# timfpark/heatmap

Hardware: AMD Instinct MI355X
Metric: points binned/sec (whole node, zooms 0-18) + % HBM roofline at 1/2/4/8 GPU (higher is better)
Workload: dtype f64

## Files before the change

heatmap_amd/csrc/hm_api.cpp:

```cpp
#include <hip/hip_runtime.h>
#include <stdio.h>
#include <stdlib.h>
#include <string.h>

#include <math.h>

#include <algorithm>
#include <chrono>
#include <vector>

#include "hm_genkey.h"
#include "hm_ctx.h"

namespace {

struct Level {
    int zc;
    int dbits;
    uint32_t nparents;
    uint64_t nchildren;
    uint32_t count = 0;
    uint32_t items = 0;
    bool out16 = false;
};
// ... 526 lines not shown
    *L = l;
}

namespace {

struct LevelOut {
    void* keys = nullptr;
    int slot_k = 0;
    HmRuns runs = {nullptr, nullptr};
    const uint32_t* parent_item_begin = nullptr;
    const uint64_t* parent_coord = nullptr;
    uint32_t nparents = 1;
    uint64_t level_keys = 0;
    uint32_t* seg = nullptr;
};

struct Level1Work {
    HmPart1Args a;
    uint32_t *rbase, *rcap;
    uint8_t* smask;
    HmL1Args ba;
    int F;
    uint32_t* hist;
    int64_t *redo_rows, *redo_cols;
    uint64_t stride;
    uint64_t total_cap;
    void* kout;
};

struct LevelWork {
    int restbits;
    bool contig;
    bool hot3;
    int sb;
    uint64_t l1_total;
    void* kout;
    uint2* runs_sh;
    uint32_t* nruns;
    uint32_t* rs_big;
    HmRsArgs ra;
    uint64_t* prefix;
};

struct CountCall {
    hm_ctx* ctx;
    const double* lat;
    const double* lon;
    const int64_t* rows;
    const int64_t* cols;
    const uint8_t* keep;
    int64_t n;
    int zmin, Z;
    uint64_t* keys_out;
    uint64_t* counts_out;
    int64_t capacity;
    int64_t* n_out;
    int64_t* xcells_out;
    int64_t xcapacity;
    int64_t* nx_out;

    hipStream_t s = nullptr;
    int zb = 0;
    int zs[HM_MAX_LEVELS];
    int L = 0;
    uint32_t ta = HM_TA;
    bool timing = false;
    uint32_t tiles_in = 0;
    bool from_tiles = false;
    uint64_t redo_cap = 0;
    bool spread = false;

    LevelOut hand;

    bool hot_on = false;
    bool hot_mid = false;
    int hz = 0;
    uint32_t nhot = 0;
    uint64_t l2_elems = 0;
    HmHotRunArgs hr = {};

    Level lv[HM_MAX_LEVELS];
    HmBuckets B[HM_MAX_LEVELS] = {};
    unsigned long long* totals[HM_MAX_LEVELS + 1];
    uint32_t nslots = 0;
    int32_t* slots = nullptr;
    uint32_t* slot_bucket = nullptr;
    HmExotic xl = {};
    uint64_t nx = 0;
    HmOut o;

    int l1_reruns = 0;
    int npart = 0;
// ... 57 lines not shown
    s = ctx->stream;
    zb = Z > HM_AG_LG ? Z - HM_AG_LG : 0;
    hz = zb;
    {
        int z = zb < HM_Z1 ? zb : HM_Z1;
        zs[L++] = z;
        while (z < zb) {
            z = std::min(z + HM_LEVEL_ZOOMS, zb);
            if (L >= HM_MAX_LEVELS) return HM_E_ARG;
            zs[L++] = z;
        }
    }
    if (2 * (Z - zs[0]) > 32) return HM_E_ARG;
    timing = n >= (1ll << 24) && ctx->stage_timing;
    while (ta > ctx->ta_min && (uint64_t)n < (uint64_t)ta * ctx->ta_items) ta >>= 1;
    for (int i = 0; i < 9; i++) ctx->stage_us[i] = 0;
    ctx->stage_us[8] = (double)ta;
    ctx->last_levels = L;

    tiles_in = (uint32_t)((n + HM_T1 - 1) / HM_T1);
    from_tiles = rows != nullptr;
    redo_cap = from_tiles ? 0 : std::max<uint64_t>(1u << 20, (uint64_t)n / 256);
    if (redo_cap > (uint64_t)n) redo_cap = (uint64_t)n;
    xl.cap = std::min<uint64_t>((uint64_t)n, std::max<uint64_t>(1u << 20, (uint64_t)n / 256));
    ENSURE(B_X_ROW, xl.cap * 8 + 8, xl.row);
    ENSURE(B_X_COL, xl.cap * 8 + 8, xl.col);
    ENSURE(B_X_IDX, xl.cap * 8 + 8, xl.idx);
    xl.count = ctx->state + ST_XCOUNT;
    return HM_OK;
}

int CountCall::begin_level(int l)
{
    Level& V = lv[l];
    V.zc = zs[l];
    V.dbits = 2 * (zs[l] - (l ? zs[l - 1] : 0));
    V.nparents = hand.nparents;
    V.nchildren = (uint64_t)hand.nparents << V.dbits;
    V.out16 = (l == L - 1);
    if (V.nchildren > (uint64_t)HM_SCAN_LIMIT) return HM_FALLBACK;
    return HM_OK;
}

int CountCall::bucket_arrays(int l, uint64_t cap, HmCompactOut& out)
{
    ENSURE(B_BK0 + l * 8 + 0, cap * 4, out.nkeys);
// ... 54 lines not shown
    const Level& V = lv[0];
    HmFill f1;
    memset(&f1, 0, sizeof(f1));
    hm_fill_add(f1, ctx->state + 1, 0, (ST_COUNT - 1) * sizeof(unsigned long long));
    hm_fill_add(f1, ctx->state + ST_ERR, 0xFF, sizeof(unsigned long long));
    static_assert(ST_ERR == 0, "error word first");
    w.F = 1 << V.dbits;
    uint32_t* fill;
    ENSURE(B_L1_FILL, FS * 4, fill);
    ENSURE(B_L1_RBASE, FS * 4, w.rbase);
    ENSURE(B_L1_RCAP, FS * 4, w.rcap);
    ENSURE(B_L1_HIST, HM_D1 * 4, w.hist);
    ENSURE(B_L1_SMASK, HM_D1, w.smask);
    uint32_t* const hist = w.hist;
    uint4* l1slot = nullptr;
    if (!from_tiles) ENSURE(B_L1_SLOT, (size_t)FS * sizeof(uint4), l1slot);
    hot_mid = ctx->hot && ctx->hot_mid && L == 3 && zs[1] <= 11 && zs[0] == HM_Z1 && n > 0 && V.dbits == 2 * HM_Z1;
    hot_on = hot_mid || (ctx->hot && L == 2 && zb <= 11 && zs[0] == HM_Z1 && n > 0 && V.dbits == 2 * HM_Z1);
    hz = hot_mid ? zs[1] : zb;
    uint32_t* redo_idx = nullptr;
    w.redo_rows = w.redo_cols = nullptr;
    if (!from_tiles) {
        ENSURE(B_REDO_IDX, redo_cap * sizeof(uint32_t), redo_idx);
        ENSURE(B_REDO_ROWS, redo_cap * sizeof(int64_t), w.redo_rows);
        ENSURE(B_REDO_COLS, redo_cap * sizeof(int64_t), w.redo_cols);
    }
    HmPart1Args& a = w.a;
    memset(&a, 0, sizeof(a));
    a.lat = lat;
    a.lon = lon;
    a.rows_in = rows;
    a.cols_in = cols;
    a.keep = keep;
    a.n = n;
    a.Z = Z;
    a.dbits = V.dbits;
    a.restbits = 2 * (Z - zs[0]);
    a.fill = fill;
    a.rbase = w.rbase;
    a.rcap = w.rcap;
    a.smask = w.smask;
    a.l1slot = l1slot;
    a.overflow = ctx->state + ST_OVERFLOW;
    a.err_word = ctx->state + ST_ERR;
    a.x = xl;
    a.slow_count = ctx->state + ST_SLOW;
    a.redo_idx = redo_idx;
    a.redo_count = ctx->state + ST_REDO;
// ... 12 lines not shown
        ENSURE(B_HOT, (HM_MAX_HOT + HM_HOT_SLOTS + 2 * HM_HOT_CAND + 1) * 4, hot_tiles);
        ENSURE(B_HOT_PARENT, HM_MAX_F1, hot_parent);
        hot_hash = hot_tiles + HM_MAX_HOT;
        hm_fill_add(f1, hot_counts, 0, 4ull << (2 * hz));
        hm_fill_add(f1, hot_hash + HM_HOT_SLOTS + 2 * HM_HOT_CAND, 0, 4);
        hm_fill_add(f1, hot_parent, 0, HM_MAX_F1);
        a.hot_z = hz;
        a.hot_bytes = hot_mid ? 4 : 2;
        a.hot_hash = hot_hash;
        a.hot_n = hot_n;
    } else {
        a.hot_z = -1;
    }
    hm_launch_fill(s, f1);
    if (n > 0) hm_launch_sample_digits(s, a, stride, hist, hot_counts);
    HIPCHK(hipGetLastError());
    if (hot_on) {
        hr.tiles = hot_tiles;
        hr.n = hot_n;
        hr.zb = hz;
        hr.z1 = zs[0];
        hr.fill = fill;
        hr.rbase = w.rbase;
        HmHotArgs ha;
        ha.counts = hot_counts;
        ha.zb = hz;
        ha.z1 = zs[0];
        const uint64_t m = ((uint64_t)n + stride - 1) / stride;
        ha.thresh = (uint32_t)std::max<double>(
            {1.0, ceil((double)m / ctx->hot_inv_share), ceil(ctx->hot_min_keys / (double)stride)});
        ha.tiles = hot_tiles;
        ha.hist = hist;
        ha.hotparent = hot_parent;
        ha.n = hot_n;
        ha.hash = hot_hash;
        ha.cand = hot_hash + HM_HOT_SLOTS;
        hm_launch_hot_select(s, ha);
        HIPCHK(hipGetLastError());
    }
    return HM_OK;
}

int CountCall::level1_size(Level1Work& w)
{
    const HmPart1Args& a = w.a;
    const int F = w.F;
    const uint64_t stride = w.stride;
    int st;
    const double nn = (double)n + (double)(F + (hot_on ? HM_MAX_HOT : 0)) * (double)stride;
    const double M = F + std::min((double)F, nn / ((double)HM_L1_SHARD_TILES * HM_T1)) * (HM_L1_SHARDS - 1) +
                     (hot_on ? (double)HM_MAX_HOT * HM_L1_SHARDS : 0.0);
    double bound = nn * 17.0 / 16.0 + 8.0 * sqrt(M * nn * (double)stride) + M * 2.0 * HM_T1 +
                   (double)(F + (hot_on ? HM_MAX_HOT : 0)) * HM_L1_ZERO_SAMPLES * (double)stride + 1024.0;
    hm_launch_l1_sizes(s, w.hist, F, hot_on ? (uint32_t*)(ctx->state + ST_NHOT) : nullptr, stride, w.rcap, w.rbase,
                       w.smask, ctx->state + ST_L1TOTAL);
    if (a.l1slot) hm_launch_l1_slots(s, a);
    HIPCHK(hipGetLastError());
    if (bound >= (double)0xFFF00000ull) {
        if ((st = read_state(ctx))) return st;
        bound = (double)ctx->host_state[ST_L1TOTAL] + 1024.0;
        if (bound >= (double)0xFFF00000ull) return HM_FALLBACK;
    }
    w.total_cap = (uint64_t)bound;
    return HM_OK;
}

int CountCall::level1_bucket_args(Level1Work& w)
{
    const Level& V = lv[0];
    HmL1Args& ba = w.ba;
    int st;
    memset(&ba, 0, sizeof(ba));
    const uint64_t cap = (uint64_t)w.F + 1;
    if ((st = bucket_arrays(0, cap, ba.out))) return st;
    ENSURE(B_FLAT_A, (uint64_t)FS * sizeof(uint2) + 8, ba.runs);
    ENSURE(B_EXCL_A, (uint64_t)FS * sizeof(uint64_t) + 8, ba.excl);
    ENSURE(B_CHILD0, 2 * 4, ba.child_begin);
    ba.F = w.F;
    ba.dbits = V.dbits;
// ... 44 lines not shown
        }
    if (w.total_cap >= 0xFFF00000ull) return HM_FALLBACK;
    HIPCHK(hipMemcpyAsync(w.rcap, hc, FS * 4, hipMemcpyHostToDevice, s));
    HIPCHK(hipMemcpyAsync(w.rbase, hb, FS * 4, hipMemcpyHostToDevice, s));
    if (a.l1slot) hm_launch_l1_slots(s, a);
    return HM_OK;
}

int CountCall::level1_redo(Level1Work& w)
{
    HmRedoArgs ra;
    ra.lat = lat;
    ra.lon = lon;
    ra.keep = keep;
    ra.Z = Z;
    ra.redo_idx = w.a.redo_idx;
    ra.redo_count = ctx->state + ST_REDO;
    ra.rows_out = w.redo_rows;
    ra.cols_out = w.redo_cols;
    ra.out_count = ctx->state + ST_REDO_OUT;
    ra.err_word = ctx->state + ST_ERR;
    ra.x = xl;
    ra.cap = redo_cap;
    hm_launch_redo(s, ra, redo_cap);
    HIPCHK(hipGetLastError());
    HmPart1Args b = w.a;
    b.lat = nullptr;
    b.lon = nullptr;
    b.rows_in = w.redo_rows;
    b.cols_in = w.redo_cols;
    b.keep = nullptr;
    b.n = (int64_t)redo_cap;
    b.n_dev = ctx->state + ST_REDO_OUT;
    hm_launch_part1(s, b, (uint32_t)((redo_cap + HM_T1 - 1) / HM_T1), lv[0].out16, 1);
    HIPCHK(hipGetLastError());
    return HM_OK;
}

int CountCall::level1_buckets(Level1Work& w)
{
    hm_launch_level1_buckets(s, w.ba);
    HIPCHK(hipGetLastError());
    if (L > 1) HIPCHK(hipMemcpyAsync(ctx->host_aux, w.hist, w.F * 4, hipMemcpyDeviceToHost, s));
    return read_state(ctx);
}

int CountCall::level1_run(Level1Work& w)
{
    const Level& V = lv[0];
    HmPart1Args& a = w.a;
    int st;
    for (int attempt = 0;; attempt++) {
        ENSURE(hand.slot_k ? B_KEYS_B : B_KEYS_A, (w.total_cap + 8) * (V.out16 ? 2 : 4), w.kout);
        a.keys_out = w.kout;
        if (hot_on) {
            void* kh = nullptr;
            if (hot_mid) l2_elems = w.total_cap + (uint64_t)n + 16;
            ENSURE(hand.slot_k ? B_KEYS_A : B_KEYS_B, hot_mid ? l2_elems * 4 : (w.total_cap + 8) * 2, kh);
            a.keys_hot = kh;
        }
        if (attempt > 0) {
            HIPCHK(hipMemsetAsync(a.fill, 0, FS * 4, s));
            static_assert(ST_XCOUNT == 1 && ST_OVERFLOW == 8 && ST_NHOT > ST_OVERFLOW, "level-1 words");
            HIPCHK(hipMemsetAsync(ctx->state + ST_XCOUNT, 0, 8 * 8, s));
        }
        if (timing) HIPCHK(hipEventRecord(ctx->ev[0], s));
        hm_launch_part1(s, a, tiles_in, V.out16, from_tiles ? 1 : 0);
        HIPCHK(hipGetLastError());
        if (timing) HIPCHK(hipEventRecord(ctx->ev[1], s));
        nev = 2;
        if (!from_tiles && (st = level1_redo(w))) return st;
        if ((st = level1_buckets(w))) return st;
        if ((st = take_error(ctx))) return st;
        const uint64_t nredo = ctx->host_state[ST_REDO];
        ctx->last_slow = (int64_t)nredo;
        if (!from_tiles && nredo > redo_cap) {
            HIPCHK(hipMemsetAsync(a.fill, 0, FS * 4, s));
            HIPCHK(hipMemsetAsync(ctx->state + ST_OVERFLOW, 0, 8, s));
            HIPCHK(hipMemsetAsync(xl.count, 0, 8, s));
            HIPCHK(hipMemsetAsync(ctx->state + ST_NSLOTS, 0, 8, s));
            HIPCHK(hipMemsetAsync(ctx->state + ST_SLOW, 0, 8, s));
            hm_launch_part1(s, a, tiles_in, V.out16, 2);
            HIPCHK(hipGetLastError());
            if ((st = level1_buckets(w))) return st;
            if ((st = take_error(ctx))) return st;
        }
        if (!ctx->host_state[ST_OVERFLOW]) break;
        if (attempt > 0) return HM_E_HIP;
        if ((st = level1_resize(w))) return st;
    }
    return HM_OK;
}

int CountCall::level1_finish(Level1Work& w)
{
    Level& V = lv[0];
    const int F = w.F;
    int st;
// ... 1156 lines not shown
```

heatmap_amd/csrc/hm_kernels.hip:

```cpp
#include <hip/hip_runtime.h>
#include "hm_genkey.h"
#include "hm_device.h"
#include "hm_project.h"
#include "hm_pipeline.h"
#define HM_STAMP_MODES(m) ((m) >= 1 && (m) <= 4)
#include "hm_stamps.h"
#include "hm_runs.h"

#define HM_YTAB_N (HM_YTAB_ROWS * HM_YTAB_STRIDE)
__constant__ double c_ytab[HM_YTAB_N] = HM_YTAB_INIT;

__device__ __forceinline__ void hm_load_ytab(double* tab)
{
    for (int i = threadIdx.x; i < HM_YTAB_N; i += blockDim.x) tab[i] = c_ytab[i];
}


__global__ __launch_bounds__(256) void k_project(const double* __restrict__ lat, const double* __restrict__ lon,
                                                 int64_t n, int zoom, int64_t* __restrict__ row,
                                                 int64_t* __restrict__ col, uint8_t* __restrict__ status,
                                                 unsigned long long* err_word, unsigned long long* slow_count)
{
    __shared__ double tab[HM_YTAB_N];
    hm_load_ytab(tab);
    __syncthreads();
    const int64_t stride = (int64_t)gridDim.x * blockDim.x;
    for (int64_t i = (int64_t)blockIdx.x * blockDim.x + threadIdx.x; i < n; i += stride) {
        int64_t r = 0, c = 0;
// ... 81 lines not shown
template <typename OutT, int MODE, bool FULL>
__global__ __launch_bounds__(HM_P1_THREADS, HM_P1_WAVES) void k_project_partition(HmPart1Args a)
{
    __shared__ uint32_t cur[HM_D1 + 64];
    __shared__ __attribute__((aligned(16))) OutT stage[HM_T1 + 64];
    __shared__ __attribute__((aligned(8))) uint16_t sdig[HM_T1 + 64];
    __shared__ unsigned long long scr[HM_P1_THREADS / 64 + 1];
    __shared__ double tab[HM_YTAB_N];
    constexpr bool HSEP = sizeof(OutT) * HM_T1 < HM_HOT_SLOTS * 4;
    constexpr bool RSEP = sizeof(uint16_t) * HM_T1 < HM_D1 * sizeof(uint2);
    __shared__ __attribute__((aligned(16))) uint32_t hsep[HSEP ? HM_HOT_SLOTS : 4];
    __shared__ __attribute__((aligned(8))) uint2 rsep[RSEP ? HM_D1 : 1];
    static_assert(sizeof(double) * HM_YTAB_N >= HM_D1 * 4, "dbase lives in the polynomial table");
    uint4* const hsh4 = HSEP ? (uint4*)hsep : (uint4*)stage;
    uint32_t* const dbase = (uint32_t*)tab;
    uint2* const rinfo = RSEP ? rsep : (uint2*)sdig;
    constexpr bool FROM_TILES = MODE == 1;
    const int tid = threadIdx.x;
    const int F = 1 << a.dbits;
    const uint32_t H = a.hot_z >= 0 ? *a.hot_n : 0u;
    const int64_t base = (a.tile0 + (int64_t)blockIdx.x) * HM_T1;
    const int64_t n = (FROM_TILES && a.n_dev) ? min((int64_t)*a.n_dev, a.n) : a.n;
    if (base >= n) return;
    if (MODE == 0) HM_STAMP_M(2, 0);
    const uint32_t lim = 1u << a.Z;
    const double scale = hm_exp2i(a.Z);
    const double kz = HM_INV360 * scale;
    uint32_t dig[HM_P1_PPT];
    uint32_t rest[HM_P1_PPT];
    int nslow = 0;
    constexpr bool FULLT = FULL && !FROM_TILES;
    double2 la[HM_P1_PPT / 2], lo[HM_P1_PPT / 2];
    uint32_t kp[HM_P1_PPT / 2];
    if (FULLT) {
        if (a.keep) {
            const uint16_t* kp2 = (const uint16_t*)(a.keep + base);
#pragma unroll
            for (int k = 0; k < HM_P1_PPT / 2; k++) kp[k] = kp2[k * HM_P1_THREADS + tid];
        } else {
#pragma unroll
            for (int k = 0; k < HM_P1_PPT / 2; k++) kp[k] = 0x0101;
        }
    }
    __builtin_amdgcn_sched_barrier(0);
    constexpr int TPT = (HM_YTAB_N + HM_P1_THREADS - 1) / HM_P1_THREADS;
    double tv[TPT];
    if (!FROM_TILES) {
// ... 63 lines not shown
            la[k] = make_double2(0.0, 0.0);
            lo[k] = make_double2(0.0, 0.0);
        }
    }
    for (int i = tid; i < HM_D1; i += HM_P1_THREADS) cur[i] = 0;
#pragma unroll
    for (int q = 0; q < PERD; q++) {
        const int d = q * HM_P1_THREADS + tid;
        const uint32_t sh = smk[q] != 0;
        rinfo[d] = make_uint2(sh ? rbase2[q][1] : rbase2[q][0], ((sh ? rcap2[q][1] : rcap2[q][0]) << 1) | sh);
    }
    if (H) {
#pragma unroll
        for (int j = 0; j < HV; j++) hsh4[j * HM_P1_THREADS + tid] = hv[j];
    }
    if (!FROM_TILES) {
#pragma unroll
        for (int q = 0; q < TPT; q++) {
            const int i = q * HM_P1_THREADS + tid;
            if (i < HM_YTAB_N) tab[i] = tv[q];
        }
    }
    __syncthreads();
    if (MODE == 0) HM_STAMP_M(2, 1);
    const int hb = a.restbits >> 1;
    const int wd = a.dbits >> 1;
    const uint32_t lowm = (1u << hb) - 1u;
    const int hs = a.Z - a.hot_z;
    const uint32_t hm = (1u << hs) - 1u;
    const uint32_t wm = (1u << wd) - 1u;
    auto key_of = [&](uint32_t r, uint32_t c, bool v, uint32_t& dslot, uint32_t& key) {
        const uint32_t rd = r >> hb, cd = c >> hb;
        uint32_t dg = (rd << wd) | (HM_SKEW_CUR ? ((cd + (rd << 3)) & wm) : cd);
        key = ((r & lowm) << hb) | (c & lowm);
        if (H) {
            const uint32_t x = hm_hot_find((const uint2*)hsh4, r >> hs, c >> hs);
            const bool hot = x < (uint32_t)HM_HOT_LIMIT;
            dg = hot ? HM_MAX_F1 + x : dg;
            key = hot ? (((r & hm) << hs) | (c & hm)) : key;
        }
        dslot = v ? dg : 0xFFFFFFFFu;
    };
    uint32_t redo = 0;
#pragma unroll
    for (int k = 0; k < HM_P1_PPT; k++) {
        const int64_t i = base + 2 * ((int64_t)(k >> 1) * HM_P1_THREADS + tid) + (k & 1);
        const double pa = (k & 1) ? la[k >> 1].y : la[k >> 1].x;
// ... 1 lines not shown
        int64_t r, c;
        int ok;
        bool dom;
        if (FROM_TILES) {
            r = __double_as_longlong(pa);
            c = __double_as_longlong(po);
            ok = 1;
            dom = ((uint64_t)r < lim) & ((uint64_t)c < lim);
        } else {
            int32_t r32, c32;
            ok = hm_project_fast(pa, po, scale, kz, &r32, &c32, tab);
            r = r32;
            c = c32;
            dom = true;
        }
        const bool inb = FULLT || i < n;
        const bool kept = ((kp[k >> 1] >> (8 * (k & 1))) & 0xFF) != 0;
        redo |= (uint32_t)(inb & !(ok & dom)) << k;
        const bool v = inb & ok & dom & kept;
        key_of((uint32_t)r, (uint32_t)c, v, dig[k], rest[k]);
        asm volatile("" : "+v"(dig[k]), "+v"(rest[k]));
        if ((k % HM_P1_ILP) == HM_P1_ILP - 1) __builtin_amdgcn_sched_barrier(0);
    }
    if (MODE == 0) HM_STAMP_M(2, 2);
    if (MODE == 0) {
        if (__ballot(redo != 0))
#pragma unroll
        for (int k = 0; k < HM_P1_PPT; k++) {
            const bool rd = (redo >> k) & 1u;
            const uint64_t m = __ballot(rd);
            if (m) {
                uint64_t b = 0;
                if (hm_lane() == __ffsll((unsigned long long)m) - 1) b = atomicAdd(a.redo_count, (unsigned long long)__popcll(m));
                b = __shfl(b, __ffsll((unsigned long long)m) - 1, 64);
                const uint64_t q = b + hm_mbcnt(m);
                if (rd && q < a.redo_cap)
                    a.redo_idx[q] = (uint32_t)(base + 2 * ((int64_t)(k >> 1) * HM_P1_THREADS + tid) + (k & 1));
            }
        }
        nslow = __popc(redo);
    } else if (__ballot(redo != 0)) {
#pragma unroll
        for (int k = 0; k < HM_P1_PPT; k++) {
            const bool rd = (redo >> k) & 1u;
            const int64_t i = base + 2 * ((int64_t)(k >> 1) * HM_P1_THREADS + tid) + (k & 1);
            int64_t r = 0, c = 0;
            int st = HM_OK;
            if (rd) {
                const double pa = (k & 1) ? la[k >> 1].y : la[k >> 1].x;
                const double po = (k & 1) ? lo[k >> 1].y : lo[k >> 1].x;
                if (FROM_TILES) {
                    r = __double_as_longlong(pa);
                    c = __double_as_longlong(po);
                } else {
                    st = hm_row_exact(pa, a.Z, &r);
                    if (st == HM_OK) st = hm_col_exact(po, a.Z, &c);
                    nslow++;
                }
            }
            const bool kept = ((kp[k >> 1] >> (8 * (k & 1))) & 0xFF) != 0;
            if (rd && st != HM_OK) atomicMin(a.err_word, ((unsigned long long)i << 8) | (unsigned long long)st);
            const bool good = rd & (st == HM_OK) & kept;
            const bool outside = good & (((uint64_t)r >= lim) | ((uint64_t)c >= lim));
            hm_exotic_append(a.x, outside, r, c, i);
            if (good & !outside) key_of((uint32_t)r, (uint32_t)c, true, dig[k], rest[k]);
        }
    }
    if (!FROM_TILES) {
        const uint32_t ws = hm_wave_sum((uint32_t)nslow);
        if (hm_lane() == 0 && ws) atomicAdd(a.slow_count, (unsigned long long)ws);
    }
    const uint32_t dummy = HM_D1 + (uint32_t)hm_lane();
    uint32_t rank[HM_P1_PPT];
#pragma unroll
    for (int k0 = 0; k0 < HM_P1_PPT; k0 += HM_P1_GROUP) {
        HmClaim gm[HM_P1_GROUP];
        uint32_t old[HM_P1_GROUP];
#pragma unroll
        for (int u = 0; u < HM_P1_GROUP; u++) {
            gm[u] = hm_claim_prep(dig[k0 + u], dig[k0 + u] != 0xFFFFFFFFu, dummy);
            old[u] = atomicAdd(&cur[gm[u].idx], gm[u].inc);
        }
#pragma unroll
        for (int u = 0; u < HM_P1_GROUP; u++) rank[k0 + u] = hm_claim_pos(gm[u], old[u]);
    }
    __syncthreads();
    if (MODE == 0) HM_STAMP_M(2, 3);
    constexpr int PER = PERD;
    uint32_t cnt[PER];
    uint32_t gpos[PER];
    uint32_t rcap[PER], rbase[PER], dsl[PER];
    uint32_t tsum = 0;
#pragma unroll
    for (int q = 0; q < PER; q++) {
        const int d = q * HM_P1_THREADS + tid;
        const uint2 ri = rinfo[d];
        rbase[q] = ri.x;
        rcap[q] = ri.y >> 1;
        dsl[q] = hm_dslot(d, wd);
        const uint32_t slot = hm_l1i(d, (ri.y & 1u) ? (blockIdx.x & (HM_L1_SHARDS - 1)) : 0u);
        cnt[q] = live(d) ? cur[dsl[q]] : 0u;
        gpos[q] = 0;
        if (cnt[q]) gpos[q] = atomicAdd(&a.fill[slot], cnt[q]);
        tsum += cnt[q];
    }
    uint32_t total;
    uint32_t offq[PER];
    offq[0] = hm_block_excl_scan<HM_P1_THREADS>(tsum, (uint32_t*)scr, &total);
#pragma unroll
    for (int q = 1; q < PER; q++) offq[q] = offq[q - 1] + cnt[q - 1];
#pragma unroll
    for (int q = 0; q < PER; q++) {
        const int d = q * HM_P1_THREADS + tid;
        if (live(d)) cur[dsl[q]] = offq[q];
    }
    __syncthreads();
    if (MODE == 0) HM_STAMP_M(2, 4);
#pragma unroll
    for (int k = 0; k < HM_P1_PPT; k++) {
        const bool v = dig[k] != 0xFFFFFFFFu;
        const uint32_t pos = v ? cur[v ? dig[k] : 0u] + rank[k] : HM_T1 + hm_lane();
        stage[pos] = (OutT)rest[k];
        sdig[pos] = (uint16_t)dig[k];
    }
    bool over = false;
#pragma unroll
    for (int q = 0; q < PER; q++) {
        const int d = q * HM_P1_THREADS + tid;
        if (live(d)) {
            const bool fits = cnt[q] && (uint64_t)gpos[q] + cnt[q] <= (uint64_t)rcap[q];
            over |= cnt[q] && !fits;
            dbase[dsl[q]] = fits ? rbase[q] + gpos[q] - offq[q] : 0xFFFFFFFFu;
        }
    }
    if (MODE == 0) HM_STAMP_M(2, 5);
    if (over) atomicOr(a.overflow, 1ull);
    __syncthreads();
    if (MODE == 0) HM_STAMP_M(2, 6);
    {
        OutT* out = (OutT*)a.keys_out;
        uint16_t* hout = (uint16_t*)a.keys_hot;
        uint32_t* hout32 = (uint32_t*)a.keys_hot;
        uint32_t sv[HM_P1_PPT], sl[HM_P1_PPT], sb[HM_P1_PPT];
#pragma unroll
        for (int j = 0; j < HM_P1_PPT; j++) {
            const uint32_t i = j * HM_P1_THREADS + tid;
            const uint32_t ic = i < total ? i : 0u;
            sl[j] = sdig[ic];
            sv[j] = (uint32_t)stage[ic];
        }
#pragma unroll
        for (int j = 0; j < HM_P1_PPT; j++) sb[j] = dbase[sl[j]];
#pragma unroll
        for (int j = 0; j < HM_P1_PPT; j++) {
            const uint32_t i = j * HM_P1_THREADS + tid;
            if (i < total && sb[j] != 0xFFFFFFFFu) {
                if (sl[j] < HM_MAX_F1)
                    out[sb[j] + i] = (OutT)sv[j];
                else if (a.hot_bytes == 4)
                    hout32[sb[j] + i] = sv[j];
                else
                    hout[sb[j] + i] = (uint16_t)sv[j];
            }
        }
    }
    if (MODE == 0) HM_STAMP_M(2, 7);
}

#ifndef HM_L1_MERGE_MIN
#define HM_L1_MERGE_MIN 6
#endif
#define HM_L1_SLOTS (HM_MAX_HOT + HM_MAX_F1)
#define HM_L1_CW 1600
static_assert(HM_L1_CW >= HM_L1_SLOTS + 64 && HM_L1_CW % 64 == 0, "count and delta words pair as read2st64");
static_assert(HM_L1_SLOTS % HM_P1_THREADS == 0, "slots per thread");

#ifndef HM_L1_WAVES
#define HM_L1_WAVES 4
#endif

__device__ __forceinline__ uint32_t hm_l1_slot_digit(uint32_t sl, int wd)
{
    if (sl < HM_MAX_HOT) return HM_MAX_F1 + sl;
    const uint32_t u = sl - HM_MAX_HOT, m = (1u << wd) - 1u;
    return HM_SKEW_CUR ? ((u & ~m) | ((u - ((u >> wd) << 3)) & m)) : u;
}
__device__ __forceinline__ bool hm_l1_slot_live(uint32_t sl, uint32_t H, uint32_t F)
{
    return sl < HM_MAX_HOT ? sl < H : (sl - HM_MAX_HOT) < F;
// ... 356 lines not shown
__global__ __launch_bounds__(256) void k_hot_select(HmHotArgs a)
{
    const uint64_t ntiles = 1ull << (2 * a.zb);
    const uint64_t stride = (uint64_t)gridDim.x * 256;
    uint32_t* const ncand = a.cand + 2 * HM_HOT_CAND;
    for (uint64_t t = (uint64_t)blockIdx.x * 256 + threadIdx.x; t < ntiles; t += stride) {
        const uint32_t c = a.counts[t];
        if (c >= a.thresh) {
            const uint32_t j = atomicAdd(ncand, 1u);
            if (j < HM_HOT_CAND) {
                a.cand[2 * j] = (uint32_t)t;
                a.cand[2 * j + 1] = c;
            }
        }
    }
}

__device__ __forceinline__ uint32_t hm_hot_bin(uint32_t c)
{
    const uint32_t e = 31u - __clz(c | 1u);
    return e < 3 ? c : (e << 3) | ((c >> (e - 3)) & 7u);
}

__global__ __launch_bounds__(1024) void k_hot_hash(HmHotArgs a)
{
    __shared__ uint32_t tab[HM_HOT_SLOTS];
    __shared__ uint32_t fill[HM_HOT_BUCKETS];
    __shared__ uint32_t bins[256];
    __shared__ uint32_t nh, cut;
    static_assert(HM_HOT_CAND <= 4 * 1024, "4 candidates a thread");
    const int tid = threadIdx.x;
    for (int i = tid; i < HM_HOT_SLOTS; i += 1024) tab[i] = HM_HOT_EMPTY;
    for (int i = tid; i < HM_HOT_BUCKETS; i += 1024) fill[i] = 0;
    for (int i = tid; i < 256; i += 1024) bins[i] = 0;
    if (tid == 0) nh = 0;
    const uint32_t nc = min(a.cand[2 * HM_HOT_CAND], (uint32_t)HM_HOT_CAND);
    uint32_t ct[4], cc[4];
#pragma unroll
    for (int u = 0; u < 4; u++) {
        const uint32_t j = tid + 1024u * u;
        const uint2 v = j < nc ? ((const uint2*)a.cand)[j] : make_uint2(0u, 0u);
        ct[u] = v.x;
        cc[u] = v.y;
    }
    __syncthreads();
#pragma unroll
    for (int u = 0; u < 4; u++)
// ... 24 lines not shown
#pragma unroll
        for (int u = 0; u < 4; u++) {
            if (tid + 1024u * u >= nc) continue;
            const uint32_t t = ct[u], c = cc[u];
            const uint32_t bn = hm_hot_bin(c);
            if (pass == 0 ? bn <= cut : pass == 1 ? bn != cut : bn >= cut) continue;
            const uint32_t tr = t >> a.zb, tc = t & ((1u << a.zb) - 1u);
            const uint32_t b = hm_hot_bucket(tr, tc);
            const uint32_t w = atomicAdd(&fill[b], 1u);
            if (w >= HM_HOT_WAYS) continue;
            const uint32_t h = atomicAdd(&nh, 1u);
            if (h >= HM_HOT_LIMIT) continue;
            tab[b * HM_HOT_WAYS + w] = (tr << HM_HOT_TAG) | h;
            a.tiles[h] = t;
            a.hist[HM_MAX_F1 + h] = c;
            const int s = a.zb - a.z1;
            const uint32_t d = ((tr >> s) << a.z1) | (tc >> s);
            a.hotparent[d] = 1;
            atomicSub(&a.hist[d], c);
        }
        __syncthreads();
    }
    for (int i = tid; i < HM_HOT_SLOTS; i += 1024) a.hash[i] = tab[i];
    if (tid == 0) *a.n = min(nh, (uint32_t)HM_HOT_LIMIT);
}

void hm_launch_hot_select(hipStream_t s, const HmHotArgs& a)
{
    const uint64_t ntiles = 1ull << (2 * a.zb);
    uint64_t blocks = (ntiles + 4095) / 4096;
    if (blocks > 1024) blocks = 1024;
    if (blocks < 1) blocks = 1;
    hipLaunchKernelGGL(k_hot_select, dim3((unsigned)blocks), dim3(256), 0, s, a);
    hipLaunchKernelGGL(k_hot_hash, dim3(1), dim3(1024), 0, s, a);
}

__device__ __forceinline__ uint32_t hm_l1_cap(uint32_t hist, uint64_t stride, int* ns)
{
    const double est = (double)hist * (double)stride;
    *ns = est > (double)HM_L1_SHARD_TILES * HM_T1 ? HM_L1_SHARDS : 1;
    const double e = est / *ns;
    return (uint32_t)fmin(1.0e9, e + e / 16 + 8.0 * sqrt(e * (double)stride) +
                                     (double)HM_L1_ZERO_SAMPLES * (double)stride / *ns + 2.0 * HM_T1);
}

__global__ __launch_bounds__(1024) void k_l1_sizes(const uint32_t* __restrict__ hist, int F,
                                                   const uint32_t* __restrict__ hot_n, uint64_t stride,
                                                   uint32_t* __restrict__ rcap, uint32_t* __restrict__ rbase,
                                                   uint8_t* __restrict__ smask, unsigned long long* total)
{
    __shared__ unsigned long long wsum[1024 / 64];
    static_assert(HM_MAX_HOT <= 1024 && HM_MAX_F1 <= 1024, "one digit of each kind per thread");
    const int t = threadIdx.x;
    const int lane = t & 63, w = t >> 6;
    const uint32_t H = hot_n ? min(*hot_n, (uint32_t)HM_MAX_HOT) : 0u;
    unsigned long long base = 0;
    for (int kind = 0; kind < 2; kind++) {
        const int d = kind ? HM_MAX_F1 + t : t;
        const bool live = kind ? (uint32_t)t < H : t < F;
        uint32_t c = 0;
        int ns = 1;
        if (live) {
            c = hm_l1_cap(hist[d], stride, &ns);
            smask[d] = (uint8_t)(ns - 1);
        }
        const unsigned long long mine = live ? (unsigned long long)c * (unsigned long long)ns : 0ull;
        unsigned long long incl = mine;
        for (int o = 1; o < 64; o <<= 1) {
            const unsigned long long y = __shfl_up(incl, o, 64);
            if (lane >= o) incl += y;
        }
        __syncthreads();
        if (lane == 63) wsum[w] = incl;
        __syncthreads();
        unsigned long long before = 0, all = 0;
        for (int i = 0; i < 1024 / 64; i++) {
            before += i < w ? wsum[i] : 0ull;
            all += wsum[i];
        }
        unsigned long long pos = base + before + incl - mine;
        if (live)
            for (int sh = 0; sh < HM_L1_SHARDS; sh++) {
                const uint32_t cs = sh < ns ? c : 0u;
                rcap[hm_l1i(d, sh)] = cs;
                rbase[hm_l1i(d, sh)] = (uint32_t)pos;
                pos += cs;
            }
        base += all;
    }
    if (t == 0 && total) *total = base;
}

void hm_launch_l1_sizes(hipStream_t s, const uint32_t* hist, int F, const uint32_t* hot_n, uint64_t stride,
                        uint32_t* rcap, uint32_t* rbase, uint8_t* smask, unsigned long long* total)
{
    hipLaunchKernelGGL(k_l1_sizes, dim3(1), dim3(1024), 0, s, hist, F, hot_n, stride, rcap, rbase, smask, total);
}

void hm_launch_sample_digits(hipStream_t s, const HmPart1Args& a, uint64_t stride_pts, uint32_t* hist,
                             uint32_t* hot_counts)
{
    const uint64_t m = ((uint64_t)a.n + stride_pts - 1) / stride_pts;
    uint64_t blocks = (m + 1023) / 1024;
    const uint64_t cap = hot_counts ? 256 : 2048;
    if (blocks > cap) blocks = cap;
    if (blocks < 1) blocks = 1;
#define HM_SD(T, H) hipLaunchKernelGGL((k_sample_digits<T, H>), dim3((unsigned)blocks), dim3(256), 0, s, a, stride_pts, \
                                       hist, hot_counts)
    if (a.rows_in) {
        if (hot_counts) HM_SD(true, true);
        else HM_SD(true, false);
    } else {
        if (hot_counts) HM_SD(false, true);
        else HM_SD(false, false);
    }
#undef HM_SD
}

__global__ __launch_bounds__(1024) void k_level1_buckets(HmL1Args a)
// ... 960 lines not shown
    f.unit[f.k] = (a % 16 == 0 && bytes % 16 == 0) ? 16u : (a % 4 == 0 && bytes % 4 == 0) ? 4u : 1u;
    f.k++;
}

void hm_launch_fill(hipStream_t s, const HmFill& f)
{
    if (!f.k) return;
    uint64_t most = 0;
    for (int e = 0; e < f.k; e++) most = std::max<uint64_t>(most, f.bytes[e] / f.unit[e]);
    hipLaunchKernelGGL(k_fill, dim3(hm_grid(most, 256, 2048)), dim3(256), 0, s, f);
}

void hm_launch_project(hipStream_t s, const double* lat, const double* lon, int64_t n, int zoom, int64_t* row,
                       int64_t* col, uint8_t* status, unsigned long long* err_word, unsigned long long* slow)
{
    const dim3 g(hm_grid(n > 0 ? (uint64_t)n : 0, 256, 256 * 16));
    hipLaunchKernelGGL(k_project, g, dim3(256), 0, s, lat, lon, n, zoom, row, col, status, err_word, slow);
}

void hm_launch_part1(hipStream_t s, const HmPart1Args& a0, uint32_t grid, bool out16, int mode)
{
    if (grid == 0) return;
    dim3 b(HM_P1_THREADS);
    const uint32_t full = mode == 1 ? 0u : (uint32_t)std::min<int64_t>(grid, a0.n / HM_T1);
    HmPart1Args a = a0;
    a.tile0 = 0;
#define HM_P1_CASE(T, M, FL, G) hipLaunchKernelGGL((k_project_partition<T, M, FL>), dim3(G), b, 0, s, a)
#define HM_P1_MODES(T, G)                             \
    do {                                              \
        if (mode == 0) HM_P1_CASE(T, 0, false, G);    \
        else if (mode == 1) HM_P1_CASE(T, 1, false, G); \
        else HM_P1_CASE(T, 2, false, G);              \
    } while (0)
    if (full) {
        if (mode == 0) {
            if (out16) {
                if (a.keep) hipLaunchKernelGGL((k_l1_fast<uint16_t, true>), dim3(full), b, 0, s, a);
                else hipLaunchKernelGGL((k_l1_fast<uint16_t, false>), dim3(full), b, 0, s, a);
            } else {
                if (a.keep) hipLaunchKernelGGL((k_l1_fast<uint32_t, true>), dim3(full), b, 0, s, a);
                else hipLaunchKernelGGL((k_l1_fast<uint32_t, false>), dim3(full), b, 0, s, a);
            }
        } else if (out16) HM_P1_CASE(uint16_t, 2, true, full);
        else HM_P1_CASE(uint32_t, 2, true, full);
    }
    if (grid > full) {
        a.tile0 = full;
        if (out16) HM_P1_MODES(uint16_t, grid - full);
        else HM_P1_MODES(uint32_t, grid - full);
    }
#undef HM_P1_MODES
#undef HM_P1_CASE
}

__global__ __launch_bounds__(256) void k_redo(HmRedoArgs a)
{
    const uint64_t n = min((uint64_t)*a.redo_count, a.cap);
    const uint64_t stride = (uint64_t)gridDim.x * blockDim.x;
    for (uint64_t q = (uint64_t)blockIdx.x * blockDim.x + threadIdx.x; q < n; q += stride) {
        const uint32_t i = a.redo_idx[q];
        int64_t r = 0, c = 0;
        int st = hm_row_exact(a.lat[i], a.Z, &r);
        if (st == HM_OK) st = hm_col_exact(a.lon[i], a.Z, &c);
        const bool kept = !a.keep || a.keep[i];
        const uint64_t lim = 1ull << a.Z;
        if (st != HM_OK) atomicMin(a.err_word, ((unsigned long long)i << 8) | (unsigned long long)st);
        const bool good = (st == HM_OK) & kept;
        const bool outside = good & (((uint64_t)r >= lim) | ((uint64_t)c >= lim));
        hm_exotic_append(a.x, outside, r, c, (int64_t)i);
        if (good & !outside) {
            const unsigned long long o = atomicAdd(a.out_count, 1ull);
            a.rows_out[o] = r;
            a.cols_out[o] = c;
        }
    }
}

void hm_launch_redo(hipStream_t s, const HmRedoArgs& a, uint64_t n)
{
    hipLaunchKernelGGL(k_redo, dim3(hm_grid(n, 256, 1024)), dim3(256), 0, s, a);
}

template <bool FROM_TILES>
__global__ __launch_bounds__(256) void k_collect_exotic(const double* lat, const double* lon, const int64_t* rows,
                                                        const int64_t* cols, const uint8_t* keep, int64_t n, int Z,
                                                        HmExotic x)
{
    __shared__ double tab[HM_YTAB_N];
    if (!FROM_TILES) hm_load_ytab(tab);
    __syncthreads();
    const uint64_t lim = 1ull << Z;
    const int64_t stride = (int64_t)gridDim.x * blockDim.x;
    const int64_t n_up = (n + 63) & ~63ll;
    for (int64_t i = (int64_t)blockIdx.x * blockDim.x + threadIdx.x; i < n_up; i += stride) {
        int64_t r = 0, c = 0;
        int st = HM_E_ARG;
// ... 309 lines not shown
```

heatmap_amd/csrc/hm_pipeline.h:

```cpp
#pragma once
#include <hip/hip_runtime.h>
#include <stdint.h>

#include "hm_top_select.h"

#ifndef HM_P1_THREADS
#define HM_P1_THREADS 512
#endif
#ifndef HM_P1_PPT
#define HM_P1_PPT 16
#endif
#define HM_T1 (HM_P1_THREADS * HM_P1_PPT)
#ifndef HM_P1_GROUP
#define HM_P1_GROUP 4
#endif
#ifndef HM_P1_ILP
#define HM_P1_ILP 1
#endif
#ifndef HM_P1_WAVES
#define HM_P1_WAVES 1
#endif
#define HM_L1_SHARDS 8
#ifndef HM_L1_SHARD_TILES
#define HM_L1_SHARD_TILES 16
// ... 341 lines not shown
    int64_t n;
    uint8_t* text;
};
void hm_launch_format_ids(hipStream_t s, const HmIdArgs& a);

#define HM_FILL_MAX 10
struct HmFill {
    void* p[HM_FILL_MAX];
    uint64_t bytes[HM_FILL_MAX];
    uint32_t word[HM_FILL_MAX];
    uint32_t unit[HM_FILL_MAX];
    int k;
};
void hm_fill_add(HmFill& f, void* p, int value, uint64_t bytes);
void hm_launch_fill(hipStream_t s, const HmFill& f);

void hm_launch_project(hipStream_t s, const double* lat, const double* lon, int64_t n, int zoom, int64_t* row,
                       int64_t* col, uint8_t* status, unsigned long long* err_word, unsigned long long* slow);
void hm_launch_part1(hipStream_t s, const HmPart1Args& a, uint32_t grid, bool out16, int mode);
void hm_launch_sample_digits(hipStream_t s, const HmPart1Args& a, uint64_t stride_pts, uint32_t* hist,
                             uint32_t* hot_counts);
void hm_launch_hot_select(hipStream_t s, const HmHotArgs& a);
void hm_launch_l1_slots(hipStream_t s, const HmPart1Args& a);
void hm_launch_l1_sizes(hipStream_t s, const uint32_t* hist, int F, const uint32_t* hot_n, uint64_t stride,
                        uint32_t* rcap, uint32_t* rbase, uint8_t* smask, unsigned long long* total);
void hm_launch_hot_nr(hipStream_t s, const HmHotRunArgs& a);
void hm_launch_hot_force(hipStream_t s, const HmHotRunArgs& a, uint8_t* force);
void hm_launch_hot_runs(hipStream_t s, const HmHotRunArgs& a);
void hm_launch_level1_buckets(hipStream_t s, const HmL1Args& a);
struct HmRedoArgs {
    const double* lat;
    const double* lon;
    const uint8_t* keep;
    int Z;
    const uint32_t* redo_idx;
    const unsigned long long* redo_count;
    uint64_t cap;
    int64_t* rows_out;
    int64_t* cols_out;
    unsigned long long* out_count;
    unsigned long long* err_word;
    HmExotic x;
};
void hm_launch_redo(hipStream_t s, const HmRedoArgs& a, uint64_t n);
void hm_launch_collect_exotic(hipStream_t s, const double* lat, const double* lon, const int64_t* rows,
                              const int64_t* cols, const uint8_t* keep, int64_t n, int Z, HmExotic x);
void hm_launch_partN(hipStream_t s, const HmPartNArgs& a, uint32_t items, bool out16, bool few_runs);
void hm_launch_rs_count(hipStream_t s, const HmRsArgs& a);
void hm_launch_rs_copy(hipStream_t s, const HmRsArgs& a);
void hm_launch_rs_keys(hipStream_t s, const HmRsArgs& a);
void hm_launch_scan(hipStream_t s, const uint64_t* v, uint64_t n, uint64_t* partial, uint64_t* out, uint64_t* total,
                    const uint64_t* ndev = nullptr);
void hm_launch_compact(hipStream_t s, const HmCompactArgs& a);
void hm_launch_items(hipStream_t s, const HmBuckets& B, HmRuns in, uint32_t items, uint32_t T, uint4* desc,
                     uint32_t* seg);
void hm_launch_aggregate(hipStream_t s, const HmAggArgs& a, uint32_t items, uint32_t nslots);
void hm_launch_small(hipStream_t s, const HmAggArgs& a, uint64_t* partial);
void hm_launch_pool(hipStream_t s, const HmPoolArgs& a, uint32_t nparents);
void hm_launch_read_stream(hipStream_t s, const void* a, const void* b, uint64_t bytes_each, uint64_t* sink);
void hm_launch_synth(hipStream_t s, int kind, uint64_t seed, int64_t start, int64_t n, double* lat, double* lon,
                     const double* tab, int k);

#define HMS_EMPTY 0xFFFFFFFFFFFFFFFFull
enum {
    HMS_ST_OCCUPIED = 0, HMS_ST_OVERFLOW = 1, HMS_ST_CURSOR = 2, HMS_ST_BUCKETS = 3, HMS_ST_BFULL = 4,
// ... 494 lines not shown
```

Baseline: 194.8 billion.

## Fold hot hashing, L1 sizing and slots into one plan kernel; route tail points through redo

Merges the hot-hash, L1 size and L1 slot-table kernels into one single-block k_l1_plan launch, which removes small serial launches from the level-1 setup path. The partial last tile is no longer handled by a mode-0 project_partition launch. Those points are now projected inside k_redo, with a fast path and an exact fallback, so level 1 only launches k_l1_fast over full tiles. Redo output writes use wave-aggregated atomics, and stamp instrumentation in mode 0 is removed. In exchange, k_l1_plan does more serial work in a single block, the redo buffers grow, and last_slow accounting moves to a device counter.

```diff
diff --git a/heatmap_amd/csrc/hm_api.cpp b/heatmap_amd/csrc/hm_api.cpp
--- a/heatmap_amd/csrc/hm_api.cpp
+++ b/heatmap_amd/csrc/hm_api.cpp
@@ -572,6 +572,7 @@
     HmL1Args ba;
     int F;
     uint32_t* hist;
+    HmHotArgs ha;
     int64_t *redo_rows, *redo_cols;
     uint64_t stride;
     uint64_t total_cap;
@@ -618,6 +619,7 @@
     uint32_t tiles_in = 0;
     bool from_tiles = false;
     uint64_t redo_cap = 0;
+    uint32_t tail_n = 0;
     bool spread = false;
 
     LevelOut hand;
@@ -721,6 +723,7 @@
     from_tiles = rows != nullptr;
     redo_cap = from_tiles ? 0 : std::max<uint64_t>(1u << 20, (uint64_t)n / 256);
     if (redo_cap > (uint64_t)n) redo_cap = (uint64_t)n;
+    tail_n = from_tiles ? 0u : (uint32_t)(n % HM_T1);
     xl.cap = std::min<uint64_t>((uint64_t)n, std::max<uint64_t>(1u << 20, (uint64_t)n / 256));
     ENSURE(B_X_ROW, xl.cap * 8 + 8, xl.row);
     ENSURE(B_X_COL, xl.cap * 8 + 8, xl.col);
@@ -821,8 +824,8 @@
     w.redo_rows = w.redo_cols = nullptr;
     if (!from_tiles) {
         ENSURE(B_REDO_IDX, redo_cap * sizeof(uint32_t), redo_idx);
-        ENSURE(B_REDO_ROWS, redo_cap * sizeof(int64_t), w.redo_rows);
-        ENSURE(B_REDO_COLS, redo_cap * sizeof(int64_t), w.redo_cols);
+        ENSURE(B_REDO_ROWS, (redo_cap + tail_n) * sizeof(int64_t), w.redo_rows);
+        ENSURE(B_REDO_COLS, (redo_cap + tail_n) * sizeof(int64_t), w.redo_cols);
     }
     HmPart1Args& a = w.a;
     memset(&a, 0, sizeof(a));
@@ -881,7 +884,7 @@
         hr.z1 = zs[0];
         hr.fill = fill;
         hr.rbase = w.rbase;
-        HmHotArgs ha;
+        HmHotArgs& ha = w.ha;
         ha.counts = hot_counts;
         ha.zb = hz;
         ha.z1 = zs[0];
@@ -911,9 +914,19 @@
                      (hot_on ? (double)HM_MAX_HOT * HM_L1_SHARDS : 0.0);
     double bound = nn * 17.0 / 16.0 + 8.0 * sqrt(M * nn * (double)stride) + M * 2.0 * HM_T1 +
                    (double)(F + (hot_on ? HM_MAX_HOT : 0)) * HM_L1_ZERO_SAMPLES * (double)stride + 1024.0;
-    hm_launch_l1_sizes(s, w.hist, F, hot_on ? (uint32_t*)(ctx->state + ST_NHOT) : nullptr, stride, w.rcap, w.rbase,
-                       w.smask, ctx->state + ST_L1TOTAL);
-    if (a.l1slot) hm_launch_l1_slots(s, a);
+    HmL1PlanArgs p;
+    memset(&p, 0, sizeof(p));
+    if (hot_on) p.hot = w.ha;
+    p.hot_on = hot_on;
+    p.hist = w.hist;
+    p.dbits = a.dbits;
+    p.stride = stride;
+    p.rcap = w.rcap;
+    p.rbase = w.rbase;
+    p.smask = w.smask;
+    p.total = ctx->state + ST_L1TOTAL;
+    p.l1slot = (uint4*)a.l1slot;
+    hm_launch_l1_plan(s, p);
     HIPCHK(hipGetLastError());
     if (bound >= (double)0xFFF00000ull) {
         if ((st = read_state(ctx))) return st;
@@ -1004,7 +1017,10 @@
     ra.err_word = ctx->state + ST_ERR;
     ra.x = xl;
     ra.cap = redo_cap;
-    hm_launch_redo(s, ra, redo_cap);
+    ra.tail0 = n - (int64_t)tail_n;
+    ra.tail_n = tail_n;
+    ra.tail_slow = ctx->state + ST_SLOW;
+    hm_launch_redo(s, ra, redo_cap + tail_n);
     HIPCHK(hipGetLastError());
     HmPart1Args b = w.a;
     b.lat = nullptr;
@@ -1012,9 +1028,9 @@
     b.rows_in = w.redo_rows;
     b.cols_in = w.redo_cols;
     b.keep = nullptr;
-    b.n = (int64_t)redo_cap;
+    b.n = (int64_t)(redo_cap + tail_n);
     b.n_dev = ctx->state + ST_REDO_OUT;
-    hm_launch_part1(s, b, (uint32_t)((redo_cap + HM_T1 - 1) / HM_T1), lv[0].out16, 1);
+    hm_launch_part1(s, b, (uint32_t)((redo_cap + tail_n + HM_T1 - 1) / HM_T1), lv[0].out16, 1);
     HIPCHK(hipGetLastError());
     return HM_OK;
 }
@@ -1055,7 +1071,6 @@
         if ((st = level1_buckets(w))) return st;
         if ((st = take_error(ctx))) return st;
         const uint64_t nredo = ctx->host_state[ST_REDO];
-        ctx->last_slow = (int64_t)nredo;
         if (!from_tiles && nredo > redo_cap) {
             HIPCHK(hipMemsetAsync(a.fill, 0, FS * 4, s));
             HIPCHK(hipMemsetAsync(ctx->state + ST_OVERFLOW, 0, 8, s));
diff --git a/heatmap_amd/csrc/hm_kernels.hip b/heatmap_amd/csrc/hm_kernels.hip
--- a/heatmap_amd/csrc/hm_kernels.hip
+++ b/heatmap_amd/csrc/hm_kernels.hip
@@ -3,7 +3,7 @@
 #include "hm_device.h"
 #include "hm_project.h"
 #include "hm_pipeline.h"
-#define HM_STAMP_MODES(m) ((m) >= 1 && (m) <= 4)
+#define HM_STAMP_MODES(m) ((m) == 1 || (m) == 3 || (m) == 4)
 #include "hm_stamps.h"
 #include "hm_runs.h"
 
@@ -131,7 +131,6 @@
     const int64_t base = (a.tile0 + (int64_t)blockIdx.x) * HM_T1;
     const int64_t n = (FROM_TILES && a.n_dev) ? min((int64_t)*a.n_dev, a.n) : a.n;
     if (base >= n) return;
-    if (MODE == 0) HM_STAMP_M(2, 0);
     const uint32_t lim = 1u << a.Z;
     const double scale = hm_exp2i(a.Z);
     const double kz = HM_INV360 * scale;
@@ -241,7 +240,6 @@
         }
     }
     __syncthreads();
-    if (MODE == 0) HM_STAMP_M(2, 1);
     const int hb = a.restbits >> 1;
     const int wd = a.dbits >> 1;
     const uint32_t lowm = (1u << hb) - 1u;
@@ -289,24 +287,7 @@
         asm volatile("" : "+v"(dig[k]), "+v"(rest[k]));
         if ((k % HM_P1_ILP) == HM_P1_ILP - 1) __builtin_amdgcn_sched_barrier(0);
     }
-    if (MODE == 0) HM_STAMP_M(2, 2);
-    if (MODE == 0) {
-        if (__ballot(redo != 0))
-#pragma unroll
-        for (int k = 0; k < HM_P1_PPT; k++) {
-            const bool rd = (redo >> k) & 1u;
-            const uint64_t m = __ballot(rd);
-            if (m) {
-                uint64_t b = 0;
-                if (hm_lane() == __ffsll((unsigned long long)m) - 1) b = atomicAdd(a.redo_count, (unsigned long long)__popcll(m));
-                b = __shfl(b, __ffsll((unsigned long long)m) - 1, 64);
-                const uint64_t q = b + hm_mbcnt(m);
-                if (rd && q < a.redo_cap)
-                    a.redo_idx[q] = (uint32_t)(base + 2 * ((int64_t)(k >> 1) * HM_P1_THREADS + tid) + (k & 1));
-            }
-        }
-        nslow = __popc(redo);
-    } else if (__ballot(redo != 0)) {
+    if (__ballot(redo != 0)) {
 #pragma unroll
         for (int k = 0; k < HM_P1_PPT; k++) {
             const bool rd = (redo >> k) & 1u;
@@ -352,7 +333,6 @@
         for (int u = 0; u < HM_P1_GROUP; u++) rank[k0 + u] = hm_claim_pos(gm[u], old[u]);
     }
     __syncthreads();
-    if (MODE == 0) HM_STAMP_M(2, 3);
     constexpr int PER = PERD;
     uint32_t cnt[PER];
     uint32_t gpos[PER];
@@ -382,7 +362,6 @@
         if (live(d)) cur[dsl[q]] = offq[q];
     }
     __syncthreads();
-    if (MODE == 0) HM_STAMP_M(2, 4);
 #pragma unroll
     for (int k = 0; k < HM_P1_PPT; k++) {
         const bool v = dig[k] != 0xFFFFFFFFu;
@@ -400,10 +379,8 @@
             dbase[dsl[q]] = fits ? rbase[q] + gpos[q] - offq[q] : 0xFFFFFFFFu;
         }
     }
-    if (MODE == 0) HM_STAMP_M(2, 5);
     if (over) atomicOr(a.overflow, 1ull);
     __syncthreads();
-    if (MODE == 0) HM_STAMP_M(2, 6);
     {
         OutT* out = (OutT*)a.keys_out;
         uint16_t* hout = (uint16_t*)a.keys_hot;
@@ -431,7 +408,6 @@
             }
         }
     }
-    if (MODE == 0) HM_STAMP_M(2, 7);
 }
 
 #ifndef HM_L1_MERGE_MIN
@@ -834,7 +810,7 @@
     return e < 3 ? c : (e << 3) | ((c >> (e - 3)) & 7u);
 }
 
-__global__ __launch_bounds__(1024) void k_hot_hash(HmHotArgs a)
+__device__ __forceinline__ uint32_t hm_hot_hash_block(const HmHotArgs& a)
 {
     __shared__ uint32_t tab[HM_HOT_SLOTS];
     __shared__ uint32_t fill[HM_HOT_BUCKETS];
@@ -905,7 +881,9 @@
         __syncthreads();
     }
     for (int i = tid; i < HM_HOT_SLOTS; i += 1024) a.hash[i] = tab[i];
-    if (tid == 0) *a.n = min(nh, (uint32_t)HM_HOT_LIMIT);
+    const uint32_t H = min(nh, (uint32_t)HM_HOT_LIMIT);
+    if (tid == 0) *a.n = H;
+    return H;
 }
 
 void hm_launch_hot_select(hipStream_t s, const HmHotArgs& a)
@@ -915,7 +893,6 @@
     if (blocks > 1024) blocks = 1024;
     if (blocks < 1) blocks = 1;
     hipLaunchKernelGGL(k_hot_select, dim3((unsigned)blocks), dim3(256), 0, s, a);
-    hipLaunchKernelGGL(k_hot_hash, dim3(1), dim3(1024), 0, s, a);
 }
 
 __device__ __forceinline__ uint32_t hm_l1_cap(uint32_t hist, uint64_t stride, int* ns)
@@ -927,16 +904,19 @@
                                      (double)HM_L1_ZERO_SAMPLES * (double)stride / *ns + 2.0 * HM_T1);
 }
 
-__global__ __launch_bounds__(1024) void k_l1_sizes(const uint32_t* __restrict__ hist, int F,
-                                                   const uint32_t* __restrict__ hot_n, uint64_t stride,
-                                                   uint32_t* __restrict__ rcap, uint32_t* __restrict__ rbase,
-                                                   uint8_t* __restrict__ smask, unsigned long long* total)
+__global__ __launch_bounds__(1024) void k_l1_plan(HmL1PlanArgs p)
 {
     __shared__ unsigned long long wsum[1024 / 64];
     static_assert(HM_MAX_HOT <= 1024 && HM_MAX_F1 <= 1024, "one digit of each kind per thread");
     const int t = threadIdx.x;
     const int lane = t & 63, w = t >> 6;
-    const uint32_t H = hot_n ? min(*hot_n, (uint32_t)HM_MAX_HOT) : 0u;
+    uint32_t H = 0;
+    if (p.hot_on) {
+        H = min(hm_hot_hash_block(p.hot), (uint32_t)HM_MAX_HOT);
+        __threadfence();
+        __syncthreads();
+    }
+    const int F = 1 << p.dbits;
     unsigned long long base = 0;
     for (int kind = 0; kind < 2; kind++) {
         const int d = kind ? HM_MAX_F1 + t : t;
@@ -944,8 +924,8 @@
         uint32_t c = 0;
         int ns = 1;
         if (live) {
-            c = hm_l1_cap(hist[d], stride, &ns);
-            smask[d] = (uint8_t)(ns - 1);
+            c = hm_l1_cap(__hip_atomic_load(p.hist + d, __ATOMIC_RELAXED, __HIP_MEMORY_SCOPE_AGENT), p.stride, &ns);
+            p.smask[d] = (uint8_t)(ns - 1);
         }
         const unsigned long long mine = live ? (unsigned long long)c * (unsigned long long)ns : 0ull;
         unsigned long long incl = mine;
@@ -961,23 +941,29 @@
             before += i < w ? wsum[i] : 0ull;
             all += wsum[i];
         }
-        unsigned long long pos = base + before + incl - mine;
+        const uint32_t pos0 = (uint32_t)(base + before + incl - mine);
         if (live)
             for (int sh = 0; sh < HM_L1_SHARDS; sh++) {
-                const uint32_t cs = sh < ns ? c : 0u;
-                rcap[hm_l1i(d, sh)] = cs;
-                rbase[hm_l1i(d, sh)] = (uint32_t)pos;
-                pos += cs;
-            }
+                p.rcap[hm_l1i(d, sh)] = sh < ns ? c : 0u;
+                p.rbase[hm_l1i(d, sh)] = pos0 + (uint32_t)min(sh, ns) * c;
+            }
+        if (p.l1slot && (kind == 0 || t < HM_MAX_HOT)) {
+            const uint32_t sl = kind ? (uint32_t)t : HM_MAX_HOT + hm_dslot((uint32_t)t, p.dbits >> 1);
+            for (int b = 0; b < HM_L1_SHARDS; b++) {
+                const uint32_t sh = ns > 1 ? (uint32_t)b : 0u;
+                p.l1slot[b * HM_D1 + sl] =
+                    live ? make_uint4(pos0 + sh * c, c, hm_l1i(d, sh), 0u) : make_uint4(0u, 0u, 0u, 0u);
+            }
+        }
         base += all;
     }
-    if (t == 0 && total) *total = base;
-}
-
-void hm_launch_l1_sizes(hipStream_t s, const uint32_t* hist, int F, const uint32_t* hot_n, uint64_t stride,
-                        uint32_t* rcap, uint32_t* rbase, uint8_t* smask, unsigned long long* total)
-{
-    hipLaunchKernelGGL(k_l1_sizes, dim3(1), dim3(1024), 0, s, hist, F, hot_n, stride, rcap, rbase, smask, total);
+    if (t == 0 && p.total) *p.total = base;
+}
+
+void hm_launch_l1_plan(hipStream_t s, const HmL1PlanArgs& p)
+{
+    static_assert(HM_D1 == HM_MAX_HOT + HM_MAX_F1, "the slot table's rows are k_l1_fast's slots");
+    hipLaunchKernelGGL(k_l1_plan, dim3(1), dim3(1024), 0, s, p);
 }
 
 void hm_launch_sample_digits(hipStream_t s, const HmPart1Args& a, uint64_t stride_pts, uint32_t* hist,
@@ -1984,56 +1970,79 @@
 {
     if (grid == 0) return;
     dim3 b(HM_P1_THREADS);
-    const uint32_t full = mode == 1 ? 0u : (uint32_t)std::min<int64_t>(grid, a0.n / HM_T1);
     HmPart1Args a = a0;
     a.tile0 = 0;
+    const uint32_t full = mode == 1 ? 0u : (uint32_t)std::min<int64_t>(grid, a0.n / HM_T1);
+    if (mode == 0) {
+        if (!full) return;
+        if (out16) {
+            if (a.keep) hipLaunchKernelGGL((k_l1_fast<uint16_t, true>), dim3(full), b, 0, s, a);
+            else hipLaunchKernelGGL((k_l1_fast<uint16_t, false>), dim3(full), b, 0, s, a);
+        } else {
+            if (a.keep) hipLaunchKernelGGL((k_l1_fast<uint32_t, true>), dim3(full), b, 0, s, a);
+            else hipLaunchKernelGGL((k_l1_fast<uint32_t, false>), dim3(full), b, 0, s, a);
+        }
+        return;
+    }
 #define HM_P1_CASE(T, M, FL, G) hipLaunchKernelGGL((k_project_partition<T, M, FL>), dim3(G), b, 0, s, a)
-#define HM_P1_MODES(T, G)                             \
-    do {                                              \
-        if (mode == 0) HM_P1_CASE(T, 0, false, G);    \
-        else if (mode == 1) HM_P1_CASE(T, 1, false, G); \
-        else HM_P1_CASE(T, 2, false, G);              \
-    } while (0)
+    if (mode == 1) {
+        if (out16) HM_P1_CASE(uint16_t, 1, false, grid);
+        else HM_P1_CASE(uint32_t, 1, false, grid);
+        return;
+    }
     if (full) {
-        if (mode == 0) {
-            if (out16) {
-                if (a.keep) hipLaunchKernelGGL((k_l1_fast<uint16_t, true>), dim3(full), b, 0, s, a);
-                else hipLaunchKernelGGL((k_l1_fast<uint16_t, false>), dim3(full), b, 0, s, a);
-            } else {
-                if (a.keep) hipLaunchKernelGGL((k_l1_fast<uint32_t, true>), dim3(full), b, 0, s, a);
-                else hipLaunchKernelGGL((k_l1_fast<uint32_t, false>), dim3(full), b, 0, s, a);
-            }
-        } else if (out16) HM_P1_CASE(uint16_t, 2, true, full);
+        if (out16) HM_P1_CASE(uint16_t, 2, true, full);
         else HM_P1_CASE(uint32_t, 2, true, full);
     }
     if (grid > full) {
         a.tile0 = full;
-        if (out16) HM_P1_MODES(uint16_t, grid - full);
-        else HM_P1_MODES(uint32_t, grid - full);
-    }
-#undef HM_P1_MODES
+        if (out16) HM_P1_CASE(uint16_t, 2, false, grid - full);
+        else HM_P1_CASE(uint32_t, 2, false, grid - full);
+    }
 #undef HM_P1_CASE
 }
 
 __global__ __launch_bounds__(256) void k_redo(HmRedoArgs a)
 {
-    const uint64_t n = min((uint64_t)*a.redo_count, a.cap);
+    const uint64_t nl = min((uint64_t)*a.redo_count, a.cap);
+    const uint64_t n = nl + a.tail_n;
     const uint64_t stride = (uint64_t)gridDim.x * blockDim.x;
+    const uint64_t lim = 1ull << a.Z;
+    const double scale = hm_exp2i(a.Z);
+    const double kz = HM_INV360 * scale;
     for (uint64_t q = (uint64_t)blockIdx.x * blockDim.x + threadIdx.x; q < n; q += stride) {
-        const uint32_t i = a.redo_idx[q];
+        const bool tail = q >= nl;
+        const int64_t i = tail ? a.tail0 + (int64_t)(q - nl) : (int64_t)a.redo_idx[q];
         int64_t r = 0, c = 0;
-        int st = hm_row_exact(a.lat[i], a.Z, &r);
-        if (st == HM_OK) st = hm_col_exact(a.lon[i], a.Z, &c);
+        bool fast = false;
+        if (tail) {
+            int32_t r32 = 0, c32 = 0;
+            fast = hm_project_fast(a.lat[i], a.lon[i], scale, kz, &r32, &c32, (const double*)c_ytab) != 0;
+            r = r32;
+            c = c32;
+            if (!fast) atomicAdd(a.tail_slow, 1ull);
+        }
+        int st = HM_OK;
+        if (!fast) {
+            st = hm_row_exact(a.lat[i], a.Z, &r);
+            if (st == HM_OK) st = hm_col_exact(a.lon[i], a.Z, &c);
+        }
         const bool kept = !a.keep || a.keep[i];
-        const uint64_t lim = 1ull << a.Z;
         if (st != HM_OK) atomicMin(a.err_word, ((unsigned long long)i << 8) | (unsigned long long)st);
         const bool good = (st == HM_OK) & kept;
         const bool outside = good & (((uint64_t)r >= lim) | ((uint64_t)c >= lim));
-        hm_exotic_append(a.x, outside, r, c, (int64_t)i);
-        if (good & !outside) {
-            const unsigned long long o = atomicAdd(a.out_count, 1ull);
-            a.rows_out[o] = r;
-            a.cols_out[o] = c;
+        hm_exotic_append(a.x, outside, r, c, i);
+        const bool put = good & !outside;
+        const uint64_t m = __ballot(put);
+        if (m) {
+            const int lead = __ffsll((unsigned long long)m) - 1;
+            unsigned long long o = 0;
+            if (hm_lane() == lead) o = atomicAdd(a.out_count, (unsigned long long)__popcll(m));
+            o = __shfl(o, lead, 64) + hm_mbcnt(m);
+            if (put) {
+                a.rows_out[o] = r;
+                a.cols_out[o] = c;
+            }
         }
     }
 }
diff --git a/heatmap_amd/csrc/hm_pipeline.h b/heatmap_amd/csrc/hm_pipeline.h
--- a/heatmap_amd/csrc/hm_pipeline.h
+++ b/heatmap_amd/csrc/hm_pipeline.h
@@ -387,8 +387,19 @@
                              uint32_t* hot_counts);
 void hm_launch_hot_select(hipStream_t s, const HmHotArgs& a);
 void hm_launch_l1_slots(hipStream_t s, const HmPart1Args& a);
-void hm_launch_l1_sizes(hipStream_t s, const uint32_t* hist, int F, const uint32_t* hot_n, uint64_t stride,
-                        uint32_t* rcap, uint32_t* rbase, uint8_t* smask, unsigned long long* total);
+struct HmL1PlanArgs {
+    HmHotArgs hot;
+    int hot_on;
+    uint32_t* hist;
+    int dbits;
+    uint64_t stride;
+    uint32_t* rcap;
+    uint32_t* rbase;
+    uint8_t* smask;
+    unsigned long long* total;
+    uint4* l1slot;
+};
+void hm_launch_l1_plan(hipStream_t s, const HmL1PlanArgs& p);
 void hm_launch_hot_nr(hipStream_t s, const HmHotRunArgs& a);
 void hm_launch_hot_force(hipStream_t s, const HmHotRunArgs& a, uint8_t* force);
 void hm_launch_hot_runs(hipStream_t s, const HmHotRunArgs& a);
@@ -406,6 +417,9 @@
     unsigned long long* out_count;
     unsigned long long* err_word;
     HmExotic x;
+    int64_t tail0;
+    uint32_t tail_n;
+    unsigned long long* tail_slow;
 };
 void hm_launch_redo(hipStream_t s, const HmRedoArgs& a, uint64_t n);
 void hm_launch_collect_exotic(hipStream_t s, const double* lat, const double* lon, const int64_t* rows,
```

Result: no change. 196.1 billion (median of 5 runs) (+0.6%).
